# clementinboittiaux/sucre

Measured on AMD Instinct MI355X. Metric: restored Mpixels/sec/GPU at 1080p, 64 neighbour views; % HBM roofline, higher is better.
Workload: dtype f32

## Files before the change

sucre_amd/csrc/experiment.h:

```cpp
#pragma once

#ifdef SUCRE_EXP_NOCOMPUTE
constexpr bool kExpNoCompute = true;
#else
constexpr bool kExpNoCompute = false;
#endif
#ifdef SUCRE_EXP_NOLOAD
constexpr bool kExpNoLoad = true;
#else
constexpr bool kExpNoLoad = false;
#endif
#ifdef SUCRE_EXP_NOSTORE
constexpr bool kExpNoStore = true;
#else
constexpr bool kExpNoStore = false;
#endif
#ifndef SUCRE_STORE_NT
#define SUCRE_STORE_NT 2
#endif
constexpr int kStoreNt = SUCRE_STORE_NT;

#ifndef SUCRE_FIT_WAVES
#define SUCRE_FIT_WAVES 5
#endif
#ifndef SUCRE_CLOSED_WAVES
#define SUCRE_CLOSED_WAVES 4
#endif

#ifndef SUCRE_MIN_STRIPS
#define SUCRE_MIN_STRIPS 4
#endif

#ifndef SUCRE_RING
#define SUCRE_RING 3
#endif
#ifndef SUCRE_DMA_POLICY
#define SUCRE_DMA_POLICY " nt"
#endif

#ifndef SUCRE_EXACT_DIV
#define SUCRE_EXACT_DIV 0
#endif
constexpr bool kExactDiv = SUCRE_EXACT_DIV != 0;

#ifndef SUCRE_EXACT_J_ADAM
#define SUCRE_EXACT_J_ADAM 0
#endif
constexpr bool kExactJAdam = SUCRE_EXACT_J_ADAM != 0;

#if !defined(SUCRE_SCALED_B)
#define SUCRE_SCALED_B 1
#endif
constexpr bool kScaledBBuilt = SUCRE_SCALED_B != 0;

#if !defined(SUCRE_PAIRED_J)
#define SUCRE_PAIRED_J 1
#endif
constexpr bool kPairedBuilt = SUCRE_PAIRED_J != 0;

#if !defined(SUCRE_STAGED_TERMS)
#define SUCRE_STAGED_TERMS 1
#endif
constexpr bool kStagedTerms = SUCRE_STAGED_TERMS != 0;

#ifdef SUCRE_EXP_WAVE_TIMES
constexpr bool kExpWaveTimes = true;
#define SUCRE_EXP_EXPORT extern "C" __attribute__((visibility("default")))
#else
constexpr bool kExpWaveTimes = false;
#define SUCRE_EXP_EXPORT [[maybe_unused]] static
#endif

#ifndef SUCRE_DEAL_FIT
#define SUCRE_DEAL_FIT 64, 50, 38, 28, 20
#endif
#ifndef SUCRE_DEAL_CLOSED
#define SUCRE_DEAL_CLOSED 64, 48, 32, 20
#endif
```

sucre_amd/csrc/fit.hip:

```cpp
#include <cstddef>
#include <type_traits>

#include "experiment.h"
#include "fit_math.h"
#include "handoff.h"

namespace sucre {

struct Water {
    float B[3], nb[3], ng[3];
};

template <class ParamAt>
__device__ __forceinline__ Water water_from(ParamAt param_at) {
    Water w;
#pragma unroll
    for (int c = 0; c < 3; ++c) {
        w.B[c] = param_at(c);
        w.nb[c] = -param_at(3 + c) * kLog2e;
        w.ng[c] = -param_at(6 + c) * kLog2e;
    }
    return w;
}
__device__ __forceinline__ Water load_water(const float *__restrict__ params) {
    return water_from([&](int i) { return params[i]; });
}

__device__ __forceinline__ float uniform_f(float x) { return __uint_as_float(__builtin_amdgcn_readfirstlane(__float_as_uint(x))); }
__device__ __forceinline__ Water load_water_uniform(const float *params) {
    Water w = load_water(params);
#pragma unroll
    for (int c = 0; c < 3; ++c) { w.B[c] = uniform_f(w.B[c]); w.nb[c] = uniform_f(w.nb[c]); w.ng[c] = uniform_f(w.ng[c]); }
    return w;
}

constexpr float kInv255 = (float)(1.0 / 255.0);

struct Acc {
    float pa[3];
    float pb[3];
    float sB[3];
    float sGZ[3];
    float cost;
};

__device__ __forceinline__ void pack_sums(float (&s)[kNumSums], const float (&sB)[3], const float (&sGZ)[3], const float (&sBeta)[3], float cost) {
#pragma unroll
    for (int c = 0; c < 3; ++c) { s[c] = sB[c]; s[3 + c] = sGZ[c]; s[6 + c] = sBeta[c]; }
    s[9] = cost;
}

struct Exps { float a[kGroupLv][3], g[kGroupLv][3]; };

__device__ __forceinline__ void chunk_exps(const float (&zz)[kGroupLv], const Water &w, Exps &e) {
#pragma unroll
    for (int j = 0; j < kGroupLv; ++j)
#pragma unroll
        for (int c = 0; c < 3; ++c) { e.a[j][c] = zz[j] * w.nb[c]; e.g[j][c] = zz[j] * w.ng[c]; }
    __builtin_amdgcn_sched_barrier(0);
#pragma unroll
    for (int j = 0; j < kGroupLv; ++j)
#pragma unroll
        for (int c = 0; c < 3; ++c) { e.a[j][c] = fast_exp2(e.a[j][c]); e.g[j][c] = fast_exp2(e.g[j][c]); }
    __builtin_amdgcn_sched_barrier(0);
}

template <bool kScaledB, bool kYield = false>
__device__ __forceinline__ void grad_terms(float z, float a, float g, uint32_t k, bool valid, float Bc, float Jc, int c, Acc &acc) {
    const float omg = kScaledB ? __builtin_fmaf(-Bc, g, Bc) : 1.0f - g;
    float Ihat = __builtin_fmaf(Jc, a, kScaledB ? omg : Bc * omg);
    if (kYield) asm volatile("s_nop 0" : "+v"(Ihat));
    float r = __builtin_fmaf((float)k, kInv255, -Ihat);
    r = valid ? r : 0.0f;
    if (kYield) asm volatile("s_nop 0" : "+v"(r));
    const float rz = r * z;
    acc.cost = __builtin_fmaf(r, r, acc.cost);
    acc.pa[c] = __builtin_fmaf(r, a, acc.pa[c]);
    acc.pb[c] = __builtin_fmaf(rz, a, acc.pb[c]);
    acc.sB[c] = __builtin_fmaf(r, omg, acc.sB[c]);
    acc.sGZ[c] = __builtin_fmaf(rz, g, acc.sGZ[c]);
    if (kYield) asm volatile("s_nop 0" : "+v"(acc.sGZ[c]));
}

template <bool kMasked, bool kScaledB, bool kYield = kStagedTerms>
__device__ __forceinline__ void accumulate_chunk(const float (&zz)[kGroupLv], const uint32_t (&cc)[3], const Water &w,
                                                 const float (&J)[3], Acc &acc) {
    if (kExpNoCompute) {
        acc.cost += (zz[0] + zz[1]) + (zz[2] + zz[3]) + (float)(cc[0] ^ cc[1] ^ cc[2]);
        return;
    }
    Exps e;
    chunk_exps(zz, w, e);
#pragma unroll
    for (int j = 0; j < kGroupLv; ++j) {
        const float z = zz[j];
        const bool valid = !kMasked || z > 0.0f;
#pragma unroll
        for (int c = 0; c < 3; ++c) grad_terms<kScaledB, kYield>(z, e.a[j][c], e.g[j][c], (cc[c] >> (8 * j)) & 255u, valid, w.B[c], J[c], c, acc);
    }
}

template <bool kScaledB>
__device__ __forceinline__ void accumulate_level(float z, const uint32_t (&k)[3], const Water &w, const float (&J)[3],
                                                 Acc &acc) {
    const bool valid = z > 0.0f;
#pragma unroll
    for (int c = 0; c < 3; ++c) grad_terms<kScaledB>(z, fast_exp2(z * w.nb[c]), fast_exp2(z * w.ng[c]), k[c], valid, w.B[c], J[c], c, acc);
}

__device__ __forceinline__ float finite_or_zero(float x) { return __builtin_isfinite(x) ? x : 0.0f; }

struct AccOne {
    float q[9][3];
};

template <bool kScaledB>
__device__ __forceinline__ void closed_terms(float z, float a, float g, uint32_t k, bool valid, float Bc, float Jp,
                                             float &q0, float &q1, float &q2, float &q3, float &q4, float &q5,
                                             float &q6, float &q7, float &q8) {
    const float omg = kScaledB ? __builtin_fmaf(-Bc, g, Bc) : 1.0f - g;
    const float y = __builtin_fmaf((float)k, kInv255, -(kScaledB ? omg : Bc * omg));
    float p = __builtin_fmaf(-Jp, a, y);
    p = valid ? p : 0.0f;
    const float za = z * a, zg = z * g;
    q0 = __builtin_fmaf(p, a, q0);
    q1 = __builtin_fmaf(a, valid ? a : 0.0f, q1);
    q2 = __builtin_fmaf(p, omg, q2);
    q3 = __builtin_fmaf(a, omg, q3);
    q4 = __builtin_fmaf(p, za, q4);
    q5 = __builtin_fmaf(a, za, q5);
    q6 = __builtin_fmaf(p, zg, q6);
    q7 = __builtin_fmaf(a, zg, q7);
    q8 = __builtin_fmaf(p, p, q8);
}

template <bool kMasked, bool kScaledB>
__device__ __forceinline__ void accumulate_chunk(const float (&zz)[kGroupLv], const uint32_t (&cc)[3], const Water &w,
                                                 const float (&Jp)[3], AccOne &acc) {
    if (kExpNoCompute) {
        acc.q[8][0] += (zz[0] + zz[1]) + (zz[2] + zz[3]) + (float)(cc[0] ^ cc[1] ^ cc[2]);
        return;
    }
    Exps e;
    chunk_exps(zz, w, e);
#pragma unroll
    for (int j = 0; j < kGroupLv; ++j) {
        const float z = zz[j];
        const bool valid = !kMasked || z > 0.0f;
#pragma unroll
        for (int c = 0; c < 3; ++c)
            closed_terms<kScaledB>(z, e.a[j][c], e.g[j][c], (cc[c] >> (8 * j)) & 255u, valid, w.B[c], Jp[c], acc.q[0][c], acc.q[1][c],
                                   acc.q[2][c], acc.q[3][c], acc.q[4][c], acc.q[5][c], acc.q[6][c], acc.q[7][c], acc.q[8][c]);
    }
}

template <bool kScaledB>
__device__ __forceinline__ void accumulate_level(float z, const uint32_t (&k)[3], const Water &w, const float (&Jp)[3],
                                                 AccOne &acc) {
    if (kExpNoCompute) {
        acc.q[8][0] += z + (float)(k[0] ^ k[1] ^ k[2]);
        return;
    }
    const bool valid = z > 0.0f;
#pragma unroll
    for (int c = 0; c < 3; ++c)
        closed_terms<kScaledB>(z, fast_exp2(z * w.nb[c]), fast_exp2(z * w.ng[c]), k[c], valid, w.B[c], Jp[c], acc.q[0][c], acc.q[1][c],
                               acc.q[2][c], acc.q[3][c], acc.q[4][c], acc.q[5][c], acc.q[6][c], acc.q[7][c], acc.q[8][c]);
}

constexpr int kRing = SUCRE_RING;
constexpr int kAhead = kRing - 1;
constexpr int kSlot = 2048;

struct __attribute__((aligned(16))) FitLds {
    uint8_t ring[4][kRing][kSlot];
    double stot[kSumsPad];
    float wsum[4][kNumSums];
    double wtotal[4][kNumSums];
    int is_last, is_last_total;
};

__device__ __forceinline__ uint32_t lds_addr(const void *p) {
    return static_cast<uint32_t>(reinterpret_cast<uintptr_t>(p));
}

static_assert(level_bytes(0) % 16 == 0 && level_bytes(1) % 16 == 0 && level_bytes(2) % 16 == 0 && level_bytes(3) % 16 == 0 && kChunk % 16 == 0 && kChunk16 % 16 == 0 && kChunk24 % 16 == 0 && kChunk26 % 16 == 0, "items are copied in 16-byte pieces");
static_assert(kChunk <= 2048 && kChunk >= 1024 && kChunk16 >= 1024 && kChunk24 >= 1024 && kChunk26 >= 1024 && kChunk26 <= kChunk, "a full chunk is one whole DMA + a partial one");
static_assert(level_bytes(0) % 64 == 0 && level_bytes(1) % 64 == 0 && level_bytes(2) % 64 == 0 && (kGroupLv * level_bytes(3)) % 64 == 0, "items start on 64-byte units (PlanItem.src64; a kStoreZ26 strip starts on a whole chunk)");

__device__ __forceinline__ void dma_item(const uint8_t *src, uint32_t slotA, uint32_t slotB, uint32_t voffA, uint32_t voffB) {
    if (kExpNoLoad) return;
    unsigned keep;
    asm volatile(
        "s_nop 4\n\t"
        "s_mov_b32 %0, m0\n\t"
        "s_mov_b32 m0, %3\n\t"
        "s_nop 0\n\t"
        "global_load_lds_dwordx4 %1, %2" SUCRE_DMA_POLICY "\n\t"
        "s_mov_b32 m0, %4\n\t"
        "s_nop 0\n\t"
        "global_load_lds_dwordx4 %5, %2" SUCRE_DMA_POLICY "\n\t"
        "s_mov_b32 m0, %0"
        : "=&s"(keep)
        : "v"(voffA), "s"(src), "s"(slotA), "s"(slotB), "v"(voffB)
        : "memory");
}

__device__ __forceinline__ void wait_vm(uint32_t n) {
#define SUCRE_W(N) case N: asm volatile("s_waitcnt vmcnt(" #N ")" ::: "memory"); break;
    switch (n) {
        SUCRE_W(0) SUCRE_W(1) SUCRE_W(2) SUCRE_W(3) SUCRE_W(4) SUCRE_W(5) SUCRE_W(6) SUCRE_W(7) SUCRE_W(8) SUCRE_W(9)
        SUCRE_W(10) SUCRE_W(11) SUCRE_W(12) SUCRE_W(13) SUCRE_W(14) SUCRE_W(15) SUCRE_W(16) SUCRE_W(17) SUCRE_W(18)
        SUCRE_W(19) SUCRE_W(20) SUCRE_W(21)
        default: asm volatile("s_waitcnt vmcnt(0)" ::: "memory"); break;
    }
#undef SUCRE_W
}
static_assert(2 * kAhead + 9 <= 63, "s_waitcnt vmcnt takes six bits");

__global__ __launch_bounds__(256) void plan_kernel(const StripMeta *__restrict__ meta, int n_strips, const uint32_t *__restrict__ store_fmt, uint32_t W0, uint32_t W1,
                                                   uint32_t Kmax, uint32_t stride0, uint32_t stride1, uint32_t kmax0, uint32_t kmax1,
                                                   PlanItem *__restrict__ plan0, PlanItem *__restrict__ plan1,
                                                   StripEntry *__restrict__ strips0, StripEntry *__restrict__ strips1,
                                                   uint32_t *__restrict__ count0, uint32_t *__restrict__ count1, uint64_t comp_off,
                                                   uint64_t state_off, uint32_t stride_pair, PlanItem *__restrict__ planL, PlanItem *__restrict__ planF,
                                                   uint64_t gplane_off) {
    const int mode = blockIdx.y;
    const int fmt = (int)store_fmt[0];
    const uint32_t W = mode ? W1 : W0, stride = mode ? stride1 : stride0, kmax = mode ? kmax1 : kmax0;
    PlanItem *plan = mode ? plan1 : plan0;
    StripEntry *strips = mode ? strips1 : strips0;
    uint32_t *count = mode ? count1 : count0;
    const uint32_t idx = blockIdx.x * 256u + threadIdx.x;
    const uint32_t wid = idx / Kmax, k = idx - wid * Kmax;
    if (wid >= W) return;
    plan_thread(mode, fmt, wid, k, W, (uint32_t)n_strips, meta, plan, strips, count, stride, kmax, comp_off, state_off, planL, planF, stride_pair, gplane_off);
}

typedef uint32_t ItemRegs __attribute__((ext_vector_type(2)));
typedef const __attribute__((address_space(4))) ItemRegs *ConstItems;

template <class T>
__device__ __forceinline__ T *uniform_ptr(T *p) {
    const uint64_t u = reinterpret_cast<uint64_t>(p);
    const uint32_t lo = __builtin_amdgcn_readfirstlane((uint32_t)u), hi = __builtin_amdgcn_readfirstlane((uint32_t)(u >> 32));
    return reinterpret_cast<T *>(((uint64_t)hi << 32) | lo);
}

template <class T>
__device__ __forceinline__ ConstItems const_items(const T *p) {
    static_assert(sizeof(T) == 8, "two dwords per entry");
    return (ConstItems)(reinterpret_cast<uintptr_t>(uniform_ptr(p)));
}

struct RangeCodes { bool z24, z26; uint32_t zoff, fullB; };

template <int kFmt>
__device__ __forceinline__ RangeCodes range_codes_of(uint32_t f0, uint32_t f1) {
    RangeCodes rc;
    rc.z24 = kFmt == 0 && f0 == (uint32_t)kStoreZ24;
    rc.z26 = kFmt == 0 && f0 == (uint32_t)kStoreZ26;
    rc.zoff = f1;
    rc.fullB = rc.z24 ? full_chunk_b(kStoreZ24) : rc.z26 ? full_chunk_b(kStoreZ26) : full_chunk_b(kFmt);
    return rc;
}

template <int kFmt>
__device__ __forceinline__ RangeCodes range_codes(const uint32_t *__restrict__ store_fmt) {
    return range_codes_of<kFmt>(__builtin_amdgcn_readfirstlane(store_fmt[0]), __builtin_amdgcn_readfirstlane(store_fmt[1]));
}

__host__ __device__ constexpr bool format_readable(int kFmt, uint32_t f) {
    return kFmt == kStoreU16 ? f == (uint32_t)kStoreU16 : (f == (uint32_t)kStoreF32 || f == (uint32_t)kStoreZ24 || f == (uint32_t)kStoreZ26);
}
template <int kFmt>
__device__ __forceinline__ bool store_matches(const uint32_t *__restrict__ store_fmt) {
    return format_readable(kFmt, __builtin_amdgcn_readfirstlane(store_fmt[0]));
}

template <int kFmt>
__device__ __forceinline__ void read_chunk(const uint8_t *sp, int lane, float (&zz)[kGroupLv], uint32_t (&cc)[3], const RangeCodes &rc, bool masked) {
    auto read_codes = [&](auto z26) {
        constexpr bool kZ26 = decltype(z26)::value;
        const uint2 a = *reinterpret_cast<const uint2 *>(sp + lane * 24), b = *reinterpret_cast<const uint2 *>(sp + lane * 24 + 8),
                    c = *reinterpret_cast<const uint2 *>(sp + lane * 24 + 16);
        const uint32_t h = kZ26 ? sp[kChunk24 + lane] : 0u;
        const uint32_t w[4] = {a.x, a.y, b.x, b.y};
#pragma unroll
        for (int j = 0; j < kGroupLv; ++j) {
            uint32_t bits;
            asm("v_mad_u32_u24 %0, %1, 1, %2" : "=v"(bits) : "v"(w[j]), "s"(rc.zoff));
            if (kZ26) bits += ((h >> (2 * j)) & 3u) << 24;
            zz[j] = __uint_as_float(bits);
            if (masked) zz[j] = (kZ26 ? bits != rc.zoff : (w[j] & 0xffffffu) != 0u) ? zz[j] : 0.0f;
        }
        cc[0] = __builtin_amdgcn_perm(a.y, a.x, 0x0c0c0703u) | __builtin_amdgcn_perm(b.y, b.x, 0x07030c0cu);
        cc[1] = c.x; cc[2] = c.y;
    };
    if (kFmt == 0 && rc.z26) return read_codes(std::true_type{});
    if (kFmt == 0 && rc.z24) return read_codes(std::false_type{});
    if (kFmt == 0) {
        const float4 z4 = *reinterpret_cast<const float4 *>(sp + lane * 16);
        zz[0] = z4.x; zz[1] = z4.y; zz[2] = z4.z; zz[3] = z4.w;
    } else {
        const uint2 q = *reinterpret_cast<const uint2 *>(sp + lane * 8);
        zz[0] = (float)(q.x & 0xffffu) * kMPerMm; zz[1] = (float)(q.x >> 16) * kMPerMm;
        zz[2] = (float)(q.y & 0xffffu) * kMPerMm; zz[3] = (float)(q.y >> 16) * kMPerMm;
    }
    const uint32_t *cp = reinterpret_cast<const uint32_t *>(sp + (kFmt ? 2 : 4) * kStripPx * kGroupLv) + 3 * lane;
    cc[0] = cp[0]; cc[1] = cp[1]; cc[2] = cp[2];
}

template <int kFmt>
__device__ __forceinline__ void read_level(const uint8_t *sp, int lane, uint32_t r, uint32_t j, float &z, uint32_t (&k)[3], const RangeCodes &rc) {
    const bool z24 = kFmt == 0 && (rc.z24 || rc.z26);
    if (z24) {
        const uint8_t *zp = sp + (lane * r + j) * 3u;
        uint32_t code = (uint32_t)zp[0] | ((uint32_t)zp[1] << 8) | ((uint32_t)zp[2] << 16);
        if (rc.z26) {
            const uint32_t f = (uint32_t)lane * r + j;
            code |= ((reinterpret_cast<const uint32_t *>(sp + 6u * kStripPx * r)[f >> 4] >> (2u * (f & 15u))) & 3u) << 24;
        }
        z = code ? __uint_as_float(code + rc.zoff) : 0.0f;
    } else if (kFmt == 0) z = reinterpret_cast<const float *>(sp)[lane * r + j];
    else z = (float)reinterpret_cast<const uint16_t *>(sp)[lane * r + j] * kMPerMm;
    const uint8_t *cb = sp + (z24 ? 3 : kFmt ? 2 : 4) * kStripPx * r;
#pragma unroll
    for (int c = 0; c < 3; ++c) k[c] = cb[c * kStripPx * r + lane * r + j];
}

template <int kFmt>
__device__ __forceinline__ void issue_item(const ItemRegs it, uint32_t ring0, uint32_t slot_off, const uint8_t *__restrict__ ws, int lane, uint32_t fullB) {
    const uint32_t lane16 = (uint32_t)lane * 16u;
    const uint32_t voffB_full = (64u + min((uint32_t)lane, fullB - 1u)) * 16u;
    const uint8_t *src = ws + ((uint64_t)it.x << 6);
    const uint32_t slot = ring0 + slot_off;
    if (it.y & kShapeFull) {
        dma_item(src, slot, slot + 1024u, lane16, voffB_full);
    } else {
        const uint32_t a_last = it.y & 127u, b_last = (it.y >> 8) & 127u, b_base = (it.y >> 16) & 127u;
        dma_item(src, slot, slot + ((a_last + 1u) << 4), min((uint32_t)lane, a_last) << 4, (b_base + min((uint32_t)lane, b_last)) << 4);
    }
}

struct NoChain { static constexpr bool kOn = false; };
struct StreamChain {
    static constexpr bool kOn = true;
    ItemRegs head[kAhead + 1], se0;
    bool next_on;
    ItemRegs next_head[kAhead];
    const uint8_t *next_ws;
    uint32_t next_fullB;
    uint32_t cs, behind;
};

template <int kFmt, int kStores, bool kMoments, bool kPrimed = false, class Chain = NoChain, int kStart = 1, class OnJ, class OnChunk, class OnTail, class OnEnd>
__device__ __forceinline__ void stream_strips(FitLds &lds, const PlanItem *__restrict__ plan, const StripEntry *__restrict__ strip_list,
                                              uint32_t K, const uint8_t *__restrict__ ws, int wave, int lane, uint32_t fullB, OnJ on_J,
                                              OnChunk on_chunk, OnTail on_tail, OnEnd on_end, Chain *chain = nullptr) {
    if (K == 0) return;
    constexpr bool kChain = Chain::kOn;
    static_assert(!kChain || kPrimed, "a chained stream's first items are in flight when it starts");
    const uint32_t ring0 = lds_addr(&lds.ring[wave][0][0]);
    const uint8_t *ringp = &lds.ring[wave][0][0];
    const ConstItems items = const_items(plan);
    const ConstItems strips = const_items(strip_list);
    uint32_t trail = 0u;
    auto issue = [&](const ItemRegs it, uint32_t slot_off) {
        if constexpr (kChain) {
            if (chain->next_on && (it.y & kShapeTrail)) {
                ItemRegs f = chain->next_head[0];
#pragma unroll
                for (int q = 1; q < kAhead; ++q) f = trail == (uint32_t)q ? chain->next_head[q] : f;
                ++trail;
                issue_item<kFmt>(f, ring0, slot_off, chain->next_ws, lane, chain->next_fullB);
                return;
            }
        }
        issue_item<kFmt>(it, ring0, slot_off, ws, lane, fullB);
    };
    if (!kPrimed) {
#pragma unroll
        for (int q = 0; q < kAhead; ++q) issue(items[q], (uint32_t)(q * kSlot));
    }
    ItemRegs nxt;
    if constexpr (kChain) nxt = chain->head[kAhead]; else nxt = items[kAhead];
    uint32_t i = 0;
    uint32_t cs = 0u;
    uint32_t behind = 0u;
    if constexpr (kChain) { cs = chain->cs; behind = chain->behind; }
    auto step = [&]() -> const uint8_t * {
        asm volatile("s_waitcnt lgkmcnt(0)" ::: "memory");
        const uint32_t is = cs == 0u ? (uint32_t)((kRing - 1) * kSlot) : cs - (uint32_t)kSlot;
        issue(nxt, is);
        nxt = items[i + (uint32_t)kAhead + 1u];
        if (behind) {
            asm volatile("s_waitcnt vmcnt(%0)" ::"n"(2 * kAhead + kStores) : "memory");
            --behind;
        } else {
            asm volatile("s_waitcnt vmcnt(%0)" ::"n"(2 * kAhead) : "memory");
        }
        const uint8_t *sp = ringp + cs;
        cs = cs == (uint32_t)((kRing - 1) * kSlot) ? 0u : cs + (uint32_t)kSlot;
        ++i;
        return sp;
    };
    ItemRegs se;
    if constexpr (kChain) se = chain->se0; else se = strips[0];
    for (uint32_t k = 0; k < K; ++k) {
        const uint32_t strip = se.x, counts = se.y;
        if (k + 1u < K) se = strips[k + 1u];
        const uint32_t nu = counts_unmasked(counts), nm = counts_masked(counts), r = counts_tail(counts);
        if constexpr (kStart == 3) {
            static_assert(!kMoments, "the moments are among the start items");
            on_J(step(), std::integral_constant<int, 0>{});
            on_J(step(), std::integral_constant<int, 1>{});
            on_J(step(), std::integral_constant<int, 2>{});
        } else {
            on_J(step());
        }
        for (uint32_t g = 0; g < nu; ++g) on_chunk(step(), false);
        for (uint32_t g = 0; g < nm; ++g) on_chunk(step(), true);
        if (r) on_tail(step(), r);
        if (kMoments) on_end(strip, step());
        else on_end(strip, (const uint8_t *)nullptr);
        behind = (uint32_t)kAhead;
    }
    if constexpr (kChain) {
        if (chain->next_on) {
            chain->cs = cs;
            chain->behind = (uint32_t)kAhead;
            return;
        }
        chain->cs = 0u;
        chain->behind = 0u;
    }
    asm volatile("s_waitcnt vmcnt(0)" ::: "memory");
}

__device__ __forceinline__ double wave_sum_fixed(double x) {
    return wave_sum_lane0(x);
}

__device__ __forceinline__ void reduce_group(const float *partials, int n_blocks, int g, double *gpart, int n_groups) {
    const int lane = threadIdx.x & 63, wave = threadIdx.x >> 6;
    const int b = g * kGroup + lane;
    for (int q = wave; q < kNumSums; q += 4) {
        double x = 0.0;
        if (lane < kGroup && b < n_blocks)
            x = (double)__hip_atomic_load(partials + (size_t)q * n_blocks + b, __ATOMIC_RELAXED, __HIP_MEMORY_SCOPE_AGENT);
        x = wave_sum_fixed(x);
        if (lane == 0) __hip_atomic_store(gpart + (size_t)q * n_groups + g, x, __ATOMIC_RELAXED, __HIP_MEMORY_SCOPE_AGENT);
    }
}

__device__ __forceinline__ double unscale_sum(double x, int q, bool scaled, float Bq) {
    return (kScaledBBuilt && scaled && q < 3) ? x / (double)Bq : x;
}

__device__ __forceinline__ void reduce_total(const double *gpart, int n_groups, double *stot, double *__restrict__ sums, const float *Bpass) {
    const int lane = threadIdx.x & 63, wave = threadIdx.x >> 6;
    const bool scaled = scaled_b_ok(Bpass[0], Bpass[1], Bpass[2]);
    for (int q = wave; q < kNumSums; q += 4) {
        double x = 0.0;
        for (int g = lane; g < n_groups; g += 64)
            x += __hip_atomic_load(gpart + (size_t)q * n_groups + g, __ATOMIC_RELAXED, __HIP_MEMORY_SCOPE_AGENT);
        x = unscale_sum(wave_sum_fixed(x), q, scaled, Bpass[q < 3 ? q : 0]);
        if (lane == 0) {
            __hip_atomic_store(sums + q, x, __ATOMIC_RELAXED, __HIP_MEMORY_SCOPE_AGENT);
            stot[q] = x;
        }
    }
    __syncthreads();
}

__device__ __forceinline__ void water_step(const double *__restrict__ sums, float *__restrict__ pstate,
                                           const uint64_t *__restrict__ n_obs_total, const AdamCoef &co,
                                           double *__restrict__ trace_row) {
    const int q = threadIdx.x & 63;
    const float scale = (1.0f / 3.0f) / (float)(*n_obs_total);
    float p = 0.f, m = 0.f, v = 0.f;
    double g = 0.0;
    if (q < 9) {
        g = water_grad(q, scale, [&](int i) { return sums[i]; }, [&](int c) { return pstate[c]; });
        p = pstate[q];
        m = pstate[9 + q];
        v = pstate[18 + q];
    }
    __builtin_amdgcn_wave_barrier();
    if (q < 9) {
        adam_update(p, m, v, (float)g, co);
        pstate[q] = p;
        pstate[9 + q] = m;
        pstate[18 + q] = v;
    }
    if (trace_row) {
        if (q < 9) trace_row[1 + q] = (double)p;
        if (q == 9) trace_row[0] = sums[9];
    }
}

__device__ __forceinline__ void wave_sums(float (&s)[kNumSums]) {
    static_assert(kNumSums == 10, "five pairs");
    float h[5];
#pragma unroll
    for (int q = 0; q < 5; ++q) {
        const auto r = __builtin_amdgcn_permlane32_swap(__float_as_uint(s[q]), __float_as_uint(s[q + 5]), false, false);
        h[q] = __uint_as_float(r[0]) + __uint_as_float(r[1]);
    }
    float R[3];
#pragma unroll
    for (int p = 0; p < 3; ++p) {
        const float a = h[2 * p], b = h[p < 2 ? 2 * p + 1 : 4];
        const auto r = __builtin_amdgcn_permlane16_swap(__float_as_uint(a), __float_as_uint(b), false, false);
        R[p] = __uint_as_float(r[0]) + __uint_as_float(r[1]);
        R[p] += lane_down<8>(R[p]);
        R[p] += lane_down<4>(R[p]);
        R[p] += lane_down<2>(R[p]);
        R[p] += lane_down<1>(R[p]);
    }
    auto at = [](float v, int lane) { return __uint_as_float(__builtin_amdgcn_readlane(__float_as_uint(v), lane)); };
    s[0] = at(R[0], 0); s[1] = at(R[0], 16); s[5] = at(R[0], 32); s[6] = at(R[0], 48);
    s[2] = at(R[1], 0); s[3] = at(R[1], 16); s[7] = at(R[1], 32); s[8] = at(R[1], 48);
    s[4] = at(R[2], 0); s[9] = at(R[2], 32);
}

template <bool kFused, bool kStep>
__device__ __forceinline__ void finish_from_wave_sums(FitLds &lds, float *partials, const AdamCoef &co, unsigned *ticket,
                                                      double *gpart, int n_groups, double *sums, float *pstate,
                                                      const uint64_t *__restrict__ n_obs_total, double *trace_row, const float *Bpass) {
    const int n_blocks = gridDim.x;
    const int t = threadIdx.x;
    __syncthreads();
    if (t < kNumSums)
        __hip_atomic_store(partials + (size_t)t * n_blocks + blockIdx.x,
                           ((lds.wsum[0][t] + lds.wsum[1][t]) + lds.wsum[2][t]) + lds.wsum[3][t], __ATOMIC_RELAXED,
                           __HIP_MEMORY_SCOPE_AGENT);

    if (kFused) {
        const int g = blockIdx.x / kGroup;
        const unsigned gsize = (unsigned)(min((g + 1) * kGroup, n_blocks) - g * kGroup);
        if (arrive_last(ticket + (size_t)(1 + g) * kTicketStride, gsize, &lds.is_last)) {
            reduce_group(partials, n_blocks, g, gpart, n_groups);
            if (arrive_last(ticket, (unsigned)n_groups, &lds.is_last_total)) {
                reduce_total(gpart, n_groups, lds.stot, sums, Bpass);
                if (kStep && t < 64) water_step(lds.stot, pstate, n_obs_total, co, trace_row);
            }
        }
    }
}

template <bool kFused, bool kStep = kFused>
__device__ __forceinline__ void finish_launch(FitLds &lds, float (&s)[kNumSums], float *partials, const AdamCoef &co,
                                              unsigned *ticket, double *gpart, int n_groups, double *sums,
                                              float *pstate, const uint64_t *__restrict__ n_obs_total,
                                              double *trace_row) {
    const int t = threadIdx.x;
    const int lane = t & 63;
    const int wave = __builtin_amdgcn_readfirstlane(t >> 6);
    wave_sums(s);
    if (lane == 0) {
#pragma unroll
        for (int q = 0; q < kNumSums; ++q) lds.wsum[wave][q] = s[q];
    }
    finish_from_wave_sums<kFused, kStep>(lds, partials, co, ticket, gpart, n_groups, sums, pstate, n_obs_total, trace_row, pstate);
}

template <class Chain>
__device__ __forceinline__ void store_stepped(float *p, float v) {
    if (kStoreNt == 1 || (kStoreNt == 2 && Chain::kOn)) __builtin_nontemporal_store(v, p);
    else *p = v;
}

template <int kFmt, bool kScaledB, bool kPrimed = false, class Chain = NoChain>
__device__ __forceinline__ void grad_pass(FitLds &lds, const PlanItem *__restrict__ plan, const StripEntry *__restrict__ strips, uint32_t n_strips_wave,
                                          const uint8_t *__restrict__ ws, float *__restrict__ state, int wave, int lane,
                                          const Water &w, float gscale, const AdamCoef &co, Acc &acc, float (&sBeta)[3], const RangeCodes &rc,
                                          Chain *chain = nullptr) {
    float J[3] = {0.f, 0.f, 0.f};
    stream_strips<kFmt, 9, true, kPrimed, Chain>(
        lds, plan, strips, n_strips_wave, ws, wave, lane, rc.fullB,
        [&](const uint8_t *sp) {
            const float *f = reinterpret_cast<const float *>(sp);
#pragma unroll
            for (int c = 0; c < 3; ++c) { J[c] = f[c * kStripPx + lane]; acc.pa[c] = 0.f; acc.pb[c] = 0.f; }
        },
        [&](const uint8_t *sp, bool masked) {
            float zz[kGroupLv];
            uint32_t cc[3];
            read_chunk<kFmt>(sp, lane, zz, cc, rc, masked);
            constexpr bool kYield = kStagedTerms && !Chain::kOn;
            if (masked) accumulate_chunk<true, kScaledB, kYield>(zz, cc, w, J, acc);
            else accumulate_chunk<false, kScaledB, kYield>(zz, cc, w, J, acc);
        },
        [&](const uint8_t *sp, uint32_t r) {
            for (uint32_t j = 0; j < r; ++j) {
                float z;
                uint32_t k[3];
                read_level<kFmt>(sp, lane, r, j, z, k, rc);
                accumulate_level<kScaledB>(z, k, w, J, acc);
            }
        },
        [&](uint32_t strip, const uint8_t *sp) {
            const float *f = reinterpret_cast<const float *>(sp);
            float *st = state + (size_t)strip * kStateFloats;
#pragma unroll
            for (int c = 0; c < 3; ++c) {
                float Jc = J[c], m = f[c * kStripPx + lane], v = f[(3 + c) * kStripPx + lane];
                sBeta[c] += (acc.pb[c] == 0.0f) ? 0.0f : Jc * acc.pb[c];
                adam_update_J(Jc, m, v, gscale * acc.pa[c], co);
                if (kExpNoStore) {
                    asm volatile("" ::"v"(Jc), "v"(m), "v"(v));
                    continue;
                }
                store_stepped<Chain>(&st[c * kStripPx + lane], Jc);
                store_stepped<Chain>(&st[(3 + c) * kStripPx + lane], m);
                store_stepped<Chain>(&st[(6 + c) * kStripPx + lane], v);
            }
        },
        chain);
}

__device__ __forceinline__ bool pass_scaled_b(const Water &w) {
    return kScaledBBuilt && __builtin_amdgcn_readfirstlane((int)scaled_b_ok(w.B[0], w.B[1], w.B[2])) != 0;
}

template <int kFmt, bool kPrimed = false, class Chain = NoChain>
__device__ __forceinline__ void run_grad_pass(bool scaled, FitLds &lds, const PlanItem *__restrict__ plan, const StripEntry *__restrict__ strips,
                                              uint32_t n_strips_wave, const uint8_t *__restrict__ ws, float *__restrict__ state, int wave, int lane,
                                              const Water &w, float gscale, const AdamCoef &co, Acc &acc, float (&sBeta)[3], const RangeCodes &rc,
                                              Chain *chain = nullptr) {
    if (kScaledBBuilt && scaled) grad_pass<kFmt, true, kPrimed, Chain>(lds, plan, strips, n_strips_wave, ws, state, wave, lane, w, gscale, co, acc, sBeta, rc, chain);
    else grad_pass<kFmt, false, kPrimed, Chain>(lds, plan, strips, n_strips_wave, ws, state, wave, lane, w, gscale, co, acc, sBeta, rc, chain);
}

template <int kFmt, bool kScaledB, int kPair>
__device__ __forceinline__ void pair_pass(FitLds &lds, const PlanItem *__restrict__ plan, const StripEntry *__restrict__ strips, uint32_t n_strips_wave,
                                          const uint8_t *__restrict__ ws, float *__restrict__ state, float *__restrict__ gplane, int wave, int lane,
                                          const Water &w, float gscale, const AdamCoef &co_prev, const AdamCoef &co, Acc &acc, float (&sBeta)[3],
                                          const RangeCodes &rc) {
    static_assert(kPair == 1 || kPair == 2, "L or F");
    float J[3] = {0.f, 0.f, 0.f}, G[3] = {0.f, 0.f, 0.f}, M[3] = {0.f, 0.f, 0.f}, V[3] = {0.f, 0.f, 0.f};
    auto begin = [&](const uint8_t *sp) {
        const float *f = reinterpret_cast<const float *>(sp);
#pragma unroll
        for (int c = 0; c < 3; ++c) { J[c] = f[c * kStripPx + lane]; acc.pa[c] = 0.f; acc.pb[c] = 0.f; }
    };
    auto on_chunk = [&](const uint8_t *sp, bool masked) {
        float zz[kGroupLv];
        uint32_t cc[3];
        read_chunk<kFmt>(sp, lane, zz, cc, rc, masked);
        if (masked) accumulate_chunk<true, kScaledB>(zz, cc, w, J, acc);
        else accumulate_chunk<false, kScaledB>(zz, cc, w, J, acc);
    };
    auto on_tail = [&](const uint8_t *sp, uint32_t r) {
        for (uint32_t j = 0; j < r; ++j) {
            float z;
            uint32_t k[3];
            read_level<kFmt>(sp, lane, r, j, z, k, rc);
            accumulate_level<kScaledB>(z, k, w, J, acc);
        }
    };
    if constexpr (kPair == 1) {
        stream_strips<kFmt, 3, false>(
            lds, plan, strips, n_strips_wave, ws, wave, lane, rc.fullB, begin, on_chunk, on_tail,
            [&](uint32_t strip, const uint8_t *) {
                float *gp = gplane + (size_t)strip * (3 * kStripPx);
#pragma unroll
                for (int c = 0; c < 3; ++c) {
                    sBeta[c] += (acc.pb[c] == 0.0f) ? 0.0f : J[c] * acc.pb[c];
                    const float g = gscale * acc.pa[c];
                    if (kExpNoStore) {
                        asm volatile("" ::"v"(g));
                        continue;
                    }
                    store_stepped<NoChain>(&gp[c * kStripPx + lane], g);
                }
            });
    } else {
        stream_strips<kFmt, 9, false, false, NoChain, 3>(
            lds, plan, strips, n_strips_wave, ws, wave, lane, rc.fullB,
            [&](const uint8_t *sp, auto which) {
                const float *f = reinterpret_cast<const float *>(sp);
                if constexpr (which.value == 0) {
                    begin(sp);
                } else if constexpr (which.value == 1) {
#pragma unroll
                    for (int c = 0; c < 3; ++c) G[c] = f[c * kStripPx + lane];
                } else {
#pragma unroll
                    for (int c = 0; c < 3; ++c) {
                        M[c] = f[c * kStripPx + lane];
                        V[c] = f[(3 + c) * kStripPx + lane];
                        adam_update_J(J[c], M[c], V[c], G[c], co_prev);
                    }
                }
            },
            on_chunk, on_tail,
            [&](uint32_t strip, const uint8_t *) {
                float *st = state + (size_t)strip * kStateFloats;
#pragma unroll
                for (int c = 0; c < 3; ++c) {
                    float Jc = J[c], m = M[c], v = V[c];
                    sBeta[c] += (acc.pb[c] == 0.0f) ? 0.0f : Jc * acc.pb[c];
                    adam_update_J(Jc, m, v, gscale * acc.pa[c], co);
                    if (kExpNoStore) {
                        asm volatile("" ::"v"(Jc), "v"(m), "v"(v));
                        continue;
                    }
                    store_stepped<NoChain>(&st[c * kStripPx + lane], Jc);
                    store_stepped<NoChain>(&st[(3 + c) * kStripPx + lane], m);
                    store_stepped<NoChain>(&st[(6 + c) * kStripPx + lane], v);
                }
            });
    }
}

__device__ __forceinline__ void zero_acc(Acc &acc) {
#pragma unroll
    for (int c = 0; c < 3; ++c) { acc.pa[c] = 0.f; acc.pb[c] = 0.f; acc.sB[c] = 0.f; acc.sGZ[c] = 0.f; }
    acc.cost = 0.f;
}

constexpr uint32_t kExpWaveSlots = 8192;
__device__ unsigned long long g_exp_wave_times[5][kExpWaveTimes ? kExpWaveSlots : 1];
}
SUCRE_EXP_EXPORT int sucre_exp_wave_times(unsigned long long *out) {
    return (int)hipMemcpyFromSymbol(out, HIP_SYMBOL(sucre::g_exp_wave_times), sizeof(sucre::g_exp_wave_times));
}
namespace sucre {

template <bool kFused, int kFmt, int kPair = 0>
__global__ __launch_bounds__(256, kFitWaves) void fit_grad_kernel(const uint8_t *__restrict__ ws,
                                                       const PlanItem *__restrict__ plan, const StripEntry *__restrict__ plan_strips, const uint32_t *__restrict__ plan_count,
                                                       uint32_t plan_stride, uint32_t plan_kmax,
                                                       float *pstate, const uint64_t *__restrict__ n_obs_total,
                                                       float *__restrict__ state, float *partials, const AdamCoef co,
                                                       unsigned *ticket, double *gpart, int n_groups, double *sums,
                                                       double *trace_row, const uint32_t *__restrict__ obs_format,
                                                       float *__restrict__ gplane, const AdamCoef co_prev) {
    __shared__ FitLds lds;
    const unsigned long long exp_t_in = kExpWaveTimes ? wall_clock64() : 0ull, exp_c_in = kExpWaveTimes ? clock64() : 0ull;
    const int t = threadIdx.x;
    const int lane = t & 63;
    const int wave = __builtin_amdgcn_readfirstlane(t >> 6);
    const Water w = load_water(pstate);
    const float gscale = -2.0f * ((1.0f / 3.0f) / (float)(*n_obs_total));
    const RangeCodes rc = range_codes<kFmt>(obs_format);
    const bool fmt_ok = store_matches<kFmt>(obs_format);
    const uint32_t wid = blockIdx.x * 4u + (uint32_t)wave;
    const uint32_t n_mine = fmt_ok ? plan_count[wid] : 0u;

    Acc acc;
    zero_acc(acc);
    if (!fmt_ok) acc.cost = __builtin_nanf("");
    float sBeta[3] = {0.f, 0.f, 0.f};
    if (kExpWaveTimes && lane == 0 && wid < kExpWaveSlots) g_exp_wave_times[0][wid] = wall_clock64();
    if constexpr (kPair == 0) {
        run_grad_pass<kFmt>(pass_scaled_b(w), lds, plan + (size_t)wid * plan_stride, plan_strips + (size_t)wid * plan_kmax, n_mine, ws, state, wave, lane, w, gscale, co, acc, sBeta, rc);
    } else {
        if (pass_scaled_b(w)) pair_pass<kFmt, true, kPair>(lds, plan + (size_t)wid * plan_stride, plan_strips + (size_t)wid * plan_kmax, n_mine, ws, state, gplane, wave, lane, w, gscale, co_prev, co, acc, sBeta, rc);
        else pair_pass<kFmt, false, kPair>(lds, plan + (size_t)wid * plan_stride, plan_strips + (size_t)wid * plan_kmax, n_mine, ws, state, gplane, wave, lane, w, gscale, co_prev, co, acc, sBeta, rc);
    }
    if (kExpWaveTimes && lane == 0 && wid < kExpWaveSlots) g_exp_wave_times[1][wid] = wall_clock64();

    float s[kNumSums];
    pack_sums(s, acc.sB, acc.sGZ, sBeta, acc.cost);
    finish_launch<kFused>(lds, s, partials, co, ticket, gpart, n_groups, sums, pstate, n_obs_total, trace_row);
    if (kExpWaveTimes && lane == 0 && wid < kExpWaveSlots) { g_exp_wave_times[2][wid] = exp_t_in; g_exp_wave_times[3][wid] = wall_clock64(); g_exp_wave_times[4][wid] = clock64() - exp_c_in; }
}

struct ClosedSums { float sB[3], sGZ[3], sBeta[3], cost; };

template <int kFmt, bool kJOnly, bool kScaledB, bool kPrimed = false, class Chain = NoChain>
__device__ __forceinline__ void closed_pass(FitLds &lds, const PlanItem *__restrict__ plan, const StripEntry *__restrict__ strips, uint32_t n_strips_wave,
                                            const uint8_t *__restrict__ ws, float *__restrict__ state, int wave, int lane,
                                            const Water &w, bool fmt_ok, ClosedSums &cs, const RangeCodes &rc, Chain *chain = nullptr) {
    AccOne acc;
    float Jp[3] = {0.f, 0.f, 0.f};
    stream_strips<kFmt, 3, false, kPrimed, Chain>(
        lds, plan, strips, n_strips_wave, ws, wave, lane, rc.fullB,
        [&](const uint8_t *sp) {
            const float *f = reinterpret_cast<const float *>(sp);
#pragma unroll
            for (int c = 0; c < 3; ++c) {
                Jp[c] = kJOnly ? 0.0f : finite_or_zero(f[c * kStripPx + lane]);
            }
#pragma unroll
            for (int q = 0; q < 9; ++q)
#pragma unroll
                for (int c = 0; c < 3; ++c) acc.q[q][c] = 0.f;
        },
        [&](const uint8_t *sp, bool masked) {
            float zz[kGroupLv];
            uint32_t cc[3];
            read_chunk<kFmt>(sp, lane, zz, cc, rc, masked);
            if (masked) accumulate_chunk<true, kScaledB>(zz, cc, w, Jp, acc);
            else accumulate_chunk<false, kScaledB>(zz, cc, w, Jp, acc);
        },
        [&](const uint8_t *sp, uint32_t r) {
            for (uint32_t j = 0; j < r; ++j) {
                float z;
                uint32_t k[3];
                read_level<kFmt>(sp, lane, r, j, z, k, rc);
                accumulate_level<kScaledB>(z, k, w, Jp, acc);
            }
        },
        [&](uint32_t strip, const uint8_t *) {
            float *st = state + (size_t)strip * kStateFloats;
#pragma unroll
            for (int c = 0; c < 3; ++c) {
                const float N = acc.q[0][c], D = acc.q[1][c];
                const float dJ = N / D;
                const float Jc = fmt_ok ? Jp[c] + dJ : __builtin_nanf("");
                store_stepped<Chain>(&st[c * kStripPx + lane], Jc);
                if (!kJOnly && D != 0.0f) {
                    cs.sB[c] += __builtin_fmaf(-dJ, acc.q[3][c], acc.q[2][c]);
                    cs.sBeta[c] += Jc * __builtin_fmaf(-dJ, acc.q[5][c], acc.q[4][c]);
                    cs.sGZ[c] += __builtin_fmaf(-dJ, acc.q[7][c], acc.q[6][c]);
                    cs.cost += __builtin_fmaf(-dJ, N, acc.q[8][c]);
                } else if (!kJOnly && N != 0.0f) {
                    cs.sB[c] += kScaledB ? dJ * w.B[c] : dJ;
                    cs.sBeta[c] += dJ;
                    cs.sGZ[c] += dJ;
                    cs.cost += __builtin_inff();
                }
            }
        },
        chain);
}

template <int kFmt, bool kPrimed = false, class Chain = NoChain>
__device__ __forceinline__ void run_closed_pass(bool scaled, FitLds &lds, const PlanItem *__restrict__ plan, const StripEntry *__restrict__ strips,
                                                uint32_t n_strips_wave, const uint8_t *__restrict__ ws, float *__restrict__ state, int wave, int lane,
                                                const Water &w, bool fmt_ok, ClosedSums &cs, const RangeCodes &rc, Chain *chain = nullptr) {
    if (kScaledBBuilt && scaled) closed_pass<kFmt, false, true, kPrimed, Chain>(lds, plan, strips, n_strips_wave, ws, state, wave, lane, w, fmt_ok, cs, rc, chain);
    else closed_pass<kFmt, false, false, kPrimed, Chain>(lds, plan, strips, n_strips_wave, ws, state, wave, lane, w, fmt_ok, cs, rc, chain);
}

template <bool kFused, int kFmt, bool kJOnly>
__global__ __launch_bounds__(256, kClosedWaves) void fit_closed_kernel(const uint8_t *__restrict__ ws,
                                                         const PlanItem *__restrict__ plan, const StripEntry *__restrict__ plan_strips, const uint32_t *__restrict__ plan_count,
                                                       uint32_t plan_stride, uint32_t plan_kmax,
                                                         float *pstate, const uint64_t *__restrict__ n_obs_total,
                                                         float *__restrict__ state, float *partials, const AdamCoef co,
                                                         unsigned *ticket, double *gpart, int n_groups, double *sums,
                                                         double *trace_row, const uint32_t *__restrict__ obs_format) {
    __shared__ FitLds lds;
    const int t = threadIdx.x;
    const int lane = t & 63;
    const int wave = __builtin_amdgcn_readfirstlane(t >> 6);
    const Water w = load_water_uniform(pstate);
    const RangeCodes rc = range_codes<kFmt>(obs_format);
    const bool fmt_ok = store_matches<kFmt>(obs_format);
    const uint32_t wid = blockIdx.x * 4u + (uint32_t)wave;
    const uint32_t n_mine = (fmt_ok || kJOnly) ? plan_count[wid] : 0u;
    ClosedSums cs = {{0.f, 0.f, 0.f}, {0.f, 0.f, 0.f}, {0.f, 0.f, 0.f}, fmt_ok ? 0.f : __builtin_nanf("")};
    if (kExpWaveTimes && !kJOnly && lane == 0 && wid < kExpWaveSlots) g_exp_wave_times[0][wid] = wall_clock64();
    if (kJOnly) closed_pass<kFmt, true, false>(lds, plan + (size_t)wid * plan_stride, plan_strips + (size_t)wid * plan_kmax, n_mine, ws, state, wave, lane, w, fmt_ok, cs, rc);
    else run_closed_pass<kFmt>(pass_scaled_b(w), lds, plan + (size_t)wid * plan_stride, plan_strips + (size_t)wid * plan_kmax, n_mine, ws, state, wave, lane, w, fmt_ok, cs, rc);
    if (kExpWaveTimes && !kJOnly && lane == 0 && wid < kExpWaveSlots) g_exp_wave_times[1][wid] = wall_clock64();
    if (kJOnly) return;
    float s[kNumSums];
    pack_sums(s, cs.sB, cs.sGZ, cs.sBeta, cs.cost);
    finish_launch<kFused>(lds, s, partials, co, ticket, gpart, n_groups, sums, pstate, n_obs_total, trace_row);
}

struct Params9 { float v[9]; };
static Params9 params9(const float *p) {
    Params9 q;
    for (int i = 0; i < 9; ++i) q.v[i] = p[i];
    return q;
}

constexpr int kGroupFitWaves = kFitWaves > 5 ? 5 : kFitWaves;

struct GroupImage {
    uint8_t *ws;
    uint64_t off_plan[2], off_strips[2], off_count[2], off_state, off_format, off_params;
    uint32_t stride[2], kmax[2], n_waves[2];
};

struct GroupHeader {
    float pstate[2][32];
    double sums[kSumsPad];
    unsigned ticket[(1 + (kFitGrid + kGroup - 1) / kGroup) * kTicketStride];
    double gpart[kNumSums * ((kFitGrid + kGroup - 1) / kGroup)];
    float partials[kNumSums * kFitGrid];
};

__host__ __device__ __forceinline__ GroupImage *group_images(GroupHeader *g) {
    return reinterpret_cast<GroupImage *>(reinterpret_cast<uint8_t *>(g) + align_up(sizeof(GroupHeader), 256));
}

__device__ __forceinline__ float ld_agent(const float *p) { return __hip_atomic_load(p, __ATOMIC_RELAXED, __HIP_MEMORY_SCOPE_AGENT); }
__device__ __forceinline__ double ld_agent(const double *p) { return __hip_atomic_load(p, __ATOMIC_RELAXED, __HIP_MEMORY_SCOPE_AGENT); }
__device__ __forceinline__ void st_agent(float *p, float v) { __hip_atomic_store(p, v, __ATOMIC_RELAXED, __HIP_MEMORY_SCOPE_AGENT); }

__device__ __forceinline__ void group_water_step(const double *__restrict__ sums, const float *__restrict__ in,
                                                 uint64_t n_obs_total, const AdamCoef &co, bool apply, float &p, float &m, float &v) {
    const int q = threadIdx.x & 63;
    p = m = v = 0.f;
    if (q < 9) {
        p = ld_agent(in + q); m = ld_agent(in + 9 + q); v = ld_agent(in + 18 + q);
        if (apply) {
            const float scale = (1.0f / 3.0f) / (float)n_obs_total;
            const double g = water_grad(q, scale, [&](int i) { return ld_agent(sums + i); }, [&](int c) { return ld_agent(in + c); });
            adam_update(p, m, v, (float)g, co);
        }
    }
}

// ... 585 lines not shown
```

Baseline: 87.96.

## Add straight-line ring-slot chunk loop with immediate-offset LDS reads for z24 ranges

```diff
diff --git a/sucre_amd/csrc/experiment.h b/sucre_amd/csrc/experiment.h
--- a/sucre_amd/csrc/experiment.h
+++ b/sucre_amd/csrc/experiment.h
@@ -63,6 +63,11 @@
 #endif
 constexpr bool kStagedTerms = SUCRE_STAGED_TERMS != 0;
 
+#if !defined(SUCRE_STRAIGHT_CHUNKS)
+#define SUCRE_STRAIGHT_CHUNKS 1
+#endif
+constexpr bool kStraightChunks = SUCRE_STRAIGHT_CHUNKS != 0 && kStagedTerms;
+
 #ifdef SUCRE_EXP_WAVE_TIMES
 constexpr bool kExpWaveTimes = true;
 #define SUCRE_EXP_EXPORT extern "C" __attribute__((visibility("default")))
diff --git a/sucre_amd/csrc/fit.hip b/sucre_amd/csrc/fit.hip
--- a/sucre_amd/csrc/fit.hip
+++ b/sucre_amd/csrc/fit.hip
@@ -106,6 +106,26 @@
     const bool valid = z > 0.0f;
 #pragma unroll
     for (int c = 0; c < 3; ++c) grad_terms<kScaledB>(z, fast_exp2(z * w.nb[c]), fast_exp2(z * w.ng[c]), k[c], valid, w.B[c], J[c], c, acc);
+}
+
+template <bool kScaledB, bool kYield>
+__device__ __forceinline__ void accumulate_chunk_z24(const float (&zz)[kGroupLv], const uint32_t (&wd)[kGroupLv], uint32_t cg, uint32_t cb,
+                                                     const Water &w, const float (&J)[3], Acc &acc) {
+    if (kExpNoCompute) {
+        acc.cost += (zz[0] + zz[1]) + (zz[2] + zz[3]) + (float)(wd[0] ^ wd[1] ^ cg ^ cb);
+        return;
+    }
+    Exps e;
+    chunk_exps(zz, w, e);
+#pragma unroll
+    for (int j = 0; j < kGroupLv; ++j) {
+        const uint32_t k[3] = {wd[j] >> 24, (cg >> (8 * j)) & 255u, (cb >> (8 * j)) & 255u};
+#pragma unroll
+        for (int c = 0; c < 3; ++c) grad_terms<kScaledB, kYield>(zz[j], e.a[j][c], e.g[j][c], k[c], true, w.B[c], J[c], c, acc);
+    }
+#pragma unroll
+    for (int c = 0; c < 3; ++c) asm volatile("" : "+v"(acc.pa[c]), "+v"(acc.pb[c]), "+v"(acc.sB[c]), "+v"(acc.sGZ[c]));
+    asm volatile("" : "+v"(acc.cost));
 }
 
 __device__ __forceinline__ float finite_or_zero(float x) { return __builtin_isfinite(x) ? x : 0.0f; }
@@ -311,6 +331,29 @@
     cc[0] = cp[0]; cc[1] = cp[1]; cc[2] = cp[2];
 }
 
+constexpr int kLaneZ24 = 24;
+template <uint32_t kOff>
+__device__ __forceinline__ void read_chunk_z24(uint32_t lane_addr, uint32_t zoff, float (&zz)[kGroupLv], uint32_t (&wd)[kGroupLv], uint32_t &cg, uint32_t &cb) {
+    static_assert(kOff + 16u < 65536u, "a ds_read offset");
+    uint64_t a, b, c;
+    asm volatile(
+        "ds_read_b64 %0, %3 offset:%4\n\t"
+        "ds_read_b64 %1, %3 offset:%5\n\t"
+        "ds_read_b64 %2, %3 offset:%6\n\t"
+        "s_waitcnt lgkmcnt(0)"
+        : "=&v"(a), "=&v"(b), "=&v"(c)
+        : "v"(lane_addr), "n"(kOff), "n"(kOff + 8u), "n"(kOff + 16u)
+        : "memory");
+    wd[0] = (uint32_t)a; wd[1] = (uint32_t)(a >> 32); wd[2] = (uint32_t)b; wd[3] = (uint32_t)(b >> 32);
+#pragma unroll
+    for (int j = 0; j < kGroupLv; ++j) {
+        uint32_t bits;
+        asm("v_mad_u32_u24 %0, %1, 1, %2" : "=v"(bits) : "v"(wd[j]), "s"(zoff));
+        zz[j] = __uint_as_float(bits);
+    }
+    cg = (uint32_t)c; cb = (uint32_t)(c >> 32);
+}
+
 template <int kFmt>
 __device__ __forceinline__ void read_level(const uint8_t *sp, int lane, uint32_t r, uint32_t j, float &z, uint32_t (&k)[3], const RangeCodes &rc) {
     const bool z24 = kFmt == 0 && (rc.z24 || rc.z26);
@@ -354,7 +397,9 @@
     uint32_t cs, behind;
 };
 
-template <int kFmt, int kStores, bool kMoments, bool kPrimed = false, class Chain = NoChain, int kStart = 1, class OnJ, class OnChunk, class OnTail, class OnEnd>
+template <uint32_t kOff> struct Straight { static constexpr uint32_t off = kOff; };
+constexpr bool kStraightRun = kStraightChunks && kRing == 3;
+template <int kFmt, int kStores, bool kMoments, bool kPrimed = false, class Chain = NoChain, int kStart = 1, int kLaneBytes = 0, class OnJ, class OnChunk, class OnTail, class OnEnd>
 __device__ __forceinline__ void stream_strips(FitLds &lds, const PlanItem *__restrict__ plan, const StripEntry *__restrict__ strip_list,
                                               uint32_t K, const uint8_t *__restrict__ ws, int wave, int lane, uint32_t fullB, OnJ on_J,
                                               OnChunk on_chunk, OnTail on_tail, OnEnd on_end, Chain *chain = nullptr) {
@@ -405,6 +450,32 @@
         ++i;
         return sp;
     };
+    constexpr bool kStraight = kLaneBytes > 0;
+    static_assert(!kStraight || !kChain, "a chained stream starts with the `behind` the previous image left");
+    static_assert(!kStraight || (kRing == 3 && kRing * kSlot <= 65536), "three slots, their offsets ds_read immediates");
+    const uint32_t lane_addr = ring0 + (uint32_t)lane * (uint32_t)kLaneBytes;
+    auto straight_step = [&](auto slot) {
+        if constexpr (kStraight) {
+            constexpr uint32_t q = decltype(slot)::value;
+            asm volatile("s_waitcnt lgkmcnt(0)" ::: "memory");
+            issue(nxt, (uint32_t)(((q + kRing - 1u) % kRing) * kSlot));
+            nxt = items[i + (uint32_t)kAhead + 1u];
+            asm volatile("s_waitcnt vmcnt(%0)" ::"n"(2 * kAhead) : "memory");
+            ++i;
+            on_chunk(lane_addr, Straight<q * kSlot>{});
+        }
+    };
+    auto straight_run = [&](uint32_t n) {
+        const std::integral_constant<uint32_t, 0> s0; const std::integral_constant<uint32_t, 1> s1; const std::integral_constant<uint32_t, 2> s2;
+        if (cs == (uint32_t)kSlot) { straight_step(s1); --n; cs = 2u * kSlot; }
+        if (cs == 2u * kSlot && n != 0u) { straight_step(s2); --n; cs = 0u; }
+        if (cs == 0u) {
+            const uint32_t turns = n / 3u, rest = n - 3u * turns;
+            for (uint32_t t = 0; t < turns; ++t) { straight_step(s0); straight_step(s1); straight_step(s2); }
+            if (rest != 0u) { straight_step(s0); cs = (uint32_t)kSlot; }
+            if (rest == 2u) { straight_step(s1); cs = 2u * kSlot; }
+        }
+    };
     ItemRegs se;
     if constexpr (kChain) se = chain->se0; else se = strips[0];
     for (uint32_t k = 0; k < K; ++k) {
@@ -419,7 +490,14 @@
         } else {
             on_J(step());
         }
-        for (uint32_t g = 0; g < nu; ++g) on_chunk(step(), false);
+        if constexpr (kStraight) {
+            constexpr uint32_t kPeel = kStart < kAhead ? (uint32_t)(kAhead - kStart) : 0u;
+            uint32_t g = 0;
+            for (; g < kPeel && g < nu; ++g) on_chunk(step(), false);
+            if (g < nu) straight_run(nu - g);
+        } else {
+            for (uint32_t g = 0; g < nu; ++g) on_chunk(step(), false);
+        }
         for (uint32_t g = 0; g < nm; ++g) on_chunk(step(), true);
         if (r) on_tail(step(), r);
         if (kMoments) on_end(strip, step());
@@ -572,32 +650,41 @@
     else *p = v;
 }
 
-template <int kFmt, bool kScaledB, bool kPrimed = false, class Chain = NoChain>
+template <int kFmt, bool kScaledB, bool kPrimed = false, class Chain = NoChain, bool kZ24 = false>
 __device__ __forceinline__ void grad_pass(FitLds &lds, const PlanItem *__restrict__ plan, const StripEntry *__restrict__ strips, uint32_t n_strips_wave,
                                           const uint8_t *__restrict__ ws, float *__restrict__ state, int wave, int lane,
                                           const Water &w, float gscale, const AdamCoef &co, Acc &acc, float (&sBeta)[3], const RangeCodes &rc,
                                           Chain *chain = nullptr) {
     float J[3] = {0.f, 0.f, 0.f};
-    stream_strips<kFmt, 9, true, kPrimed, Chain>(
+    static_assert(!kZ24 || kFmt == 0, "range codes stand for float32 ranges");
+    const RangeCodes rc24 = {true, false, rc.zoff, rc.fullB};
+    const RangeCodes &rz = kZ24 ? rc24 : rc;
+    constexpr bool kYield = kStagedTerms && !Chain::kOn;
+    stream_strips<kFmt, 9, true, kPrimed, Chain, 1, kZ24 ? kLaneZ24 : 0>(
         lds, plan, strips, n_strips_wave, ws, wave, lane, rc.fullB,
         [&](const uint8_t *sp) {
             const float *f = reinterpret_cast<const float *>(sp);
 #pragma unroll
             for (int c = 0; c < 3; ++c) { J[c] = f[c * kStripPx + lane]; acc.pa[c] = 0.f; acc.pb[c] = 0.f; }
         },
-        [&](const uint8_t *sp, bool masked) {
+        [&](auto sp, auto how) {
             float zz[kGroupLv];
-            uint32_t cc[3];
-            read_chunk<kFmt>(sp, lane, zz, cc, rc, masked);
-            constexpr bool kYield = kStagedTerms && !Chain::kOn;
-            if (masked) accumulate_chunk<true, kScaledB, kYield>(zz, cc, w, J, acc);
-            else accumulate_chunk<false, kScaledB, kYield>(zz, cc, w, J, acc);
+            if constexpr (!std::is_same_v<decltype(how), bool>) {
+                uint32_t wd[kGroupLv], cg, cb;
+                read_chunk_z24<decltype(how)::off>(sp, rz.zoff, zz, wd, cg, cb);
+                accumulate_chunk_z24<kScaledB, kYield>(zz, wd, cg, cb, w, J, acc);
+            } else {
+                uint32_t cc[3];
+                read_chunk<kFmt>(sp, lane, zz, cc, rz, how);
+                if (how) accumulate_chunk<true, kScaledB, kYield>(zz, cc, w, J, acc);
+                else accumulate_chunk<false, kScaledB, kYield>(zz, cc, w, J, acc);
+            }
         },
         [&](const uint8_t *sp, uint32_t r) {
             for (uint32_t j = 0; j < r; ++j) {
                 float z;
                 uint32_t k[3];
-                read_level<kFmt>(sp, lane, r, j, z, k, rc);
+                read_level<kFmt>(sp, lane, r, j, z, k, rz);
                 accumulate_level<kScaledB>(z, k, w, J, acc);
             }
         },
@@ -625,44 +712,61 @@
     return kScaledBBuilt && __builtin_amdgcn_readfirstlane((int)scaled_b_ok(w.B[0], w.B[1], w.B[2])) != 0;
 }
 
-template <int kFmt, bool kPrimed = false, class Chain = NoChain>
+template <int kFmt, bool kPrimed = false, class Chain = NoChain, bool kPickZ24 = false>
 __device__ __forceinline__ void run_grad_pass(bool scaled, FitLds &lds, const PlanItem *__restrict__ plan, const StripEntry *__restrict__ strips,
                                               uint32_t n_strips_wave, const uint8_t *__restrict__ ws, float *__restrict__ state, int wave, int lane,
                                               const Water &w, float gscale, const AdamCoef &co, Acc &acc, float (&sBeta)[3], const RangeCodes &rc,
                                               Chain *chain = nullptr) {
+    if constexpr (kPickZ24) {
+        if (rc.z24) {
+            if (kScaledBBuilt && scaled) grad_pass<kFmt, true, kPrimed, Chain, true>(lds, plan, strips, n_strips_wave, ws, state, wave, lane, w, gscale, co, acc, sBeta, rc, chain);
+            else grad_pass<kFmt, false, kPrimed, Chain, true>(lds, plan, strips, n_strips_wave, ws, state, wave, lane, w, gscale, co, acc, sBeta, rc, chain);
+            return;
+        }
+    }
     if (kScaledBBuilt && scaled) grad_pass<kFmt, true, kPrimed, Chain>(lds, plan, strips, n_strips_wave, ws, state, wave, lane, w, gscale, co, acc, sBeta, rc, chain);
     else grad_pass<kFmt, false, kPrimed, Chain>(lds, plan, strips, n_strips_wave, ws, state, wave, lane, w, gscale, co, acc, sBeta, rc, chain);
 }
 
-template <int kFmt, bool kScaledB, int kPair>
+template <int kFmt, bool kScaledB, int kPair, bool kZ24 = false>
 __device__ __forceinline__ void pair_pass(FitLds &lds, const PlanItem *__restrict__ plan, const StripEntry *__restrict__ strips, uint32_t n_strips_wave,
                                           const uint8_t *__restrict__ ws, float *__restrict__ state, float *__restrict__ gplane, int wave, int lane,
                                           const Water &w, float gscale, const AdamCoef &co_prev, const AdamCoef &co, Acc &acc, float (&sBeta)[3],
                                           const RangeCodes &rc) {
     static_assert(kPair == 1 || kPair == 2, "L or F");
     float J[3] = {0.f, 0.f, 0.f}, G[3] = {0.f, 0.f, 0.f}, M[3] = {0.f, 0.f, 0.f}, V[3] = {0.f, 0.f, 0.f};
+    static_assert(!kZ24 || kFmt == 0, "range codes stand for float32 ranges");
+    const RangeCodes rc24 = {true, false, rc.zoff, rc.fullB};
+    const RangeCodes &rz = kZ24 ? rc24 : rc;
+    constexpr int kLaneBytes = kZ24 ? kLaneZ24 : 0;
     auto begin = [&](const uint8_t *sp) {
         const float *f = reinterpret_cast<const float *>(sp);
 #pragma unroll
         for (int c = 0; c < 3; ++c) { J[c] = f[c * kStripPx + lane]; acc.pa[c] = 0.f; acc.pb[c] = 0.f; }
     };
-    auto on_chunk = [&](const uint8_t *sp, bool masked) {
+    auto on_chunk = [&](auto sp, auto how) {
         float zz[kGroupLv];
-        uint32_t cc[3];
-        read_chunk<kFmt>(sp, lane, zz, cc, rc, masked);
-        if (masked) accumulate_chunk<true, kScaledB>(zz, cc, w, J, acc);
-        else accumulate_chunk<false, kScaledB>(zz, cc, w, J, acc);
+        if constexpr (!std::is_same_v<decltype(how), bool>) {
+            uint32_t wd[kGroupLv], cg, cb;
+            read_chunk_z24<decltype(how)::off>(sp, rz.zoff, zz, wd, cg, cb);
+            accumulate_chunk_z24<kScaledB, kStagedTerms>(zz, wd, cg, cb, w, J, acc);
+        } else {
+            uint32_t cc[3];
+            read_chunk<kFmt>(sp, lane, zz, cc, rz, how);
+            if (how) accumulate_chunk<true, kScaledB>(zz, cc, w, J, acc);
+            else accumulate_chunk<false, kScaledB>(zz, cc, w, J, acc);
+        }
     };
     auto on_tail = [&](const uint8_t *sp, uint32_t r) {
         for (uint32_t j = 0; j < r; ++j) {
             float z;
             uint32_t k[3];
-            read_level<kFmt>(sp, lane, r, j, z, k, rc);
+            read_level<kFmt>(sp, lane, r, j, z, k, rz);
             accumulate_level<kScaledB>(z, k, w, J, acc);
         }
     };
     if constexpr (kPair == 1) {
-        stream_strips<kFmt, 3, false>(
+        stream_strips<kFmt, 3, false, false, NoChain, 1, kLaneBytes>(
             lds, plan, strips, n_strips_wave, ws, wave, lane, rc.fullB, begin, on_chunk, on_tail,
             [&](uint32_t strip, const uint8_t *) {
                 float *gp = gplane + (size_t)strip * (3 * kStripPx);
@@ -678,7 +782,7 @@
                 }
             });
     } else {
-        stream_strips<kFmt, 9, false, false, NoChain, 3>(
+        stream_strips<kFmt, 9, false, false, NoChain, 3, kLaneBytes>(
             lds, plan, strips, n_strips_wave, ws, wave, lane, rc.fullB,
             [&](const uint8_t *sp, auto which) {
                 const float *f = reinterpret_cast<const float *>(sp);
@@ -757,7 +861,11 @@
     float sBeta[3] = {0.f, 0.f, 0.f};
     if (kExpWaveTimes && lane == 0 && wid < kExpWaveSlots) g_exp_wave_times[0][wid] = wall_clock64();
     if constexpr (kPair == 0) {
-        run_grad_pass<kFmt>(pass_scaled_b(w), lds, plan + (size_t)wid * plan_stride, plan_strips + (size_t)wid * plan_kmax, n_mine, ws, state, wave, lane, w, gscale, co, acc, sBeta, rc);
+        run_grad_pass<kFmt, false, NoChain, kStraightRun && kFmt == 0>(pass_scaled_b(w), lds, plan + (size_t)wid * plan_stride, plan_strips + (size_t)wid * plan_kmax, n_mine, ws, state, wave, lane, w, gscale, co, acc, sBeta, rc);
+    } else if (kStraightRun && kFmt == 0 && rc.z24) {
+        constexpr bool kZ24 = kStraightRun && kFmt == 0;
+        if (pass_scaled_b(w)) pair_pass<kFmt, true, kPair, kZ24>(lds, plan + (size_t)wid * plan_stride, plan_strips + (size_t)wid * plan_kmax, n_mine, ws, state, gplane, wave, lane, w, gscale, co_prev, co, acc, sBeta, rc);
+        else pair_pass<kFmt, false, kPair, kZ24>(lds, plan + (size_t)wid * plan_stride, plan_strips + (size_t)wid * plan_kmax, n_mine, ws, state, gplane, wave, lane, w, gscale, co_prev, co, acc, sBeta, rc);
     } else {
         if (pass_scaled_b(w)) pair_pass<kFmt, true, kPair>(lds, plan + (size_t)wid * plan_stride, plan_strips + (size_t)wid * plan_kmax, n_mine, ws, state, gplane, wave, lane, w, gscale, co_prev, co, acc, sBeta, rc);
         else pair_pass<kFmt, false, kPair>(lds, plan + (size_t)wid * plan_stride, plan_strips + (size_t)wid * plan_kmax, n_mine, ws, state, gplane, wave, lane, w, gscale, co_prev, co, acc, sBeta, rc);
```

Result: faster. 89.64 (median of 6 runs) (+1.9%).
